# arnauqb/GradABM-JUNE

Hardware: AMD Instinct MI355X
Metric: simulation steps/sec (higher is better)
Workload: dtype f32

## Files before the change

gradabm-june_amd/csrc/gj_tiled.h:

```cpp
#pragma once
#include <hip/hip_runtime.h>
#include <stdint.h>

#include <type_traits>

#include "../../include/gradjune_hip.h"
#include "gj_device.h"

namespace gj {

constexpr int kTileThreads = 1024;
constexpr int kTileWaves = kTileThreads / kWave;
constexpr int kMaxSliceAgents = 19840;
constexpr int kUnroll = 8;
#ifndef GJ_UNROLL_NARROW
#define GJ_UNROLL_NARROW 16
#endif
constexpr int kUnrollNarrow = GJ_UNROLL_NARROW;
#ifndef GJ_VENUE_UNROLL
#define GJ_VENUE_UNROLL 2
#endif
constexpr int kVenueUnroll = GJ_VENUE_UNROLL;
#ifndef GJ_VENUE_UNROLL_C
#define GJ_VENUE_UNROLL_C GJ_VENUE_UNROLL
#endif
constexpr int kVenueUnrollC = GJ_VENUE_UNROLL_C;
#ifndef GJ_CUM_BATCH
#define GJ_CUM_BATCH 8
#endif
constexpr int kCumBatch = GJ_CUM_BATCH;

typedef unsigned long long fx_t;
template <int BITS>
__device__ __forceinline__ constexpr float fx_max() { return (float)(1ull << (50 - BITS)); }
template <int BITS>
__device__ __forceinline__ fx_t to_fx(float x) {
  constexpr double scale = (double)(1ull << BITS);
  constexpr double magic = 6755399441055744.0;
  const double d = __builtin_fma((double)x, scale, magic);
  return (fx_t)(__double_as_longlong(d) - 0x4338000000000000LL);
}
template <int BITS>
__device__ __forceinline__ float from_fx(fx_t v) {
  return (float)((double)(long long)v * (1.0 / (double)(1ull << BITS)));
}
constexpr float kSaturated = 1.0e30f;
__device__ __forceinline__ void fx_flag(uint32_t* flags, int words, int i, float x) {
  const uint32_t bit = 1u << (i & 31);
  if (!(x < 0.0f)) atomicOr(&flags[i >> 5], bit);
  if (!(x > 0.0f)) atomicOr(&flags[words + (i >> 5)], bit);
}
__device__ __forceinline__ float fx_special(uint32_t pos, uint32_t neg, float v) {
  return (pos & neg) ? __builtin_nanf("") : (pos ? kSaturated : (neg ? -kSaturated : v));
}
template <int BITS>
__device__ __forceinline__ float fx_read(const fx_t* sums, const uint32_t* flags, int words, int i) {
  const uint32_t pos = (flags[i >> 5] >> (i & 31)) & 1u, neg = (flags[words + (i >> 5)] >> (i & 31)) & 1u;
  return fx_special(pos, neg, from_fx<BITS>(sums[i]));
}
constexpr int kFxVenue = 36, kFxAgent = 32;
__device__ __forceinline__ uint32_t abs_bits(float x) { return __float_as_uint(x) & 0x7FFFFFFFu; }
template <int N>
__device__ __forceinline__ uint32_t max_abs_bits(const float (&x)[N]) {
  uint32_t m = 0u;
#pragma unroll
  for (int q = 0; q < N; ++q) m = max(m, abs_bits(x[q]));
  return m;
}
template <int BITS>
constexpr uint32_t fx_limit_bits() { return (uint32_t)(127 + 50 - BITS) << 23; }
constexpr uint32_t kAgentLimitBits = fx_limit_bits<kFxAgent>();
static_assert(kAgentLimitBits == 0x48800000u, "the pattern of fx_max<kFxAgent>() = 262144.0f");

template <typename T>
__device__ __forceinline__ T* elem32(T* base, int idx) {
  using Byte = typename std::conditional<std::is_const<T>::value, const char, char>::type;
  return reinterpret_cast<T*>(reinterpret_cast<Byte*>(base) + (uint64_t)((uint32_t)idx * (uint32_t)sizeof(T)));
}
template <typename T>
__device__ __forceinline__ T at32(const T* base, int idx) { return *elem32(base, idx); }
template <typename T>
__device__ __forceinline__ void put32(T* base, int idx, T v) { *elem32(base, idx) = v; }

typedef float gj_v4f __attribute__((ext_vector_type(4)));
typedef unsigned int gj_v4u __attribute__((ext_vector_type(4)));
typedef unsigned int gj_v2u __attribute__((ext_vector_type(2)));
template <typename T>
__device__ __forceinline__ T at32nt(const T* base, int idx) { return __builtin_nontemporal_load(elem32(base, idx)); }
template <typename T>
__device__ __forceinline__ void put32nt(T* base, int idx, T v) { __builtin_nontemporal_store(v, elem32(base, idx)); }
__device__ __forceinline__ uint4 load_nt(const uint4* p) {
  const gj_v4u v = __builtin_nontemporal_load(reinterpret_cast<const gj_v4u*>(p));
  return make_uint4(v.x, v.y, v.z, v.w);
}
__device__ __forceinline__ float4 load_nt(const float4* p) {
  const gj_v4f v = __builtin_nontemporal_load(reinterpret_cast<const gj_v4f*>(p));
  return make_float4(v.x, v.y, v.z, v.w);
}
__device__ __forceinline__ void store_nt(float4* p, float4 x) {
  gj_v4f v = {x.x, x.y, x.z, x.w};
  __builtin_nontemporal_store(v, reinterpret_cast<gj_v4f*>(p));
}
struct TSetA {
  const uint16_t* a_la;
  const int32_t* tile_sptr;
  const int32_t* tile_jpos;
  const int32_t* chunk_ptr;
  const int4* chunk_desc;
  float* val;
  int32_t J;
  int32_t active;
  int32_t raw;
  int32_t wide;
  int32_t direct;
  int32_t presum;
  const int32_t* multi_slots;
};

struct TileAArgs {
  TSetA sets[GJ_MAX_SETS];
  int32_t n_sets;
  int32_t slice_agents;
  int64_t n_agents;
  const float* trans;
  const float* qtrans;
};

__device__ __forceinline__ void load_slice(float* lds, const float* __restrict__ src, int64_t base, int n_local,
                                           int tid) {
  const int n4 = n_local >> 2;
  const float4* s4 = reinterpret_cast<const float4*>(src + base);
  float4* d4 = reinterpret_cast<float4*>(lds);
  constexpr int kQ = (kMaxSliceAgents + 4 * kTileThreads - 1) / (4 * kTileThreads);
  if (n4 > 0) {
    float4 v[kQ];
#pragma unroll
    for (int u = 0; u < kQ; ++u) v[u] = s4[min(tid + u * kTileThreads, n4 - 1)];
#pragma unroll
    for (int u = 0; u < kQ; ++u)
      if (tid + u * kTileThreads < n4) d4[tid + u * kTileThreads] = v[u];
  }
  for (int i = (n4 << 2) + tid; i < n_local; i += kTileThreads) lds[i] = src[base + i];
}

__device__ __forceinline__ int chunk_slot_fast(const int4 d, int lane) {
  const int split = d.z & 0xFFFF;
  return (lane < split) ? d.x + lane : d.y + (lane - split);
}
__device__ __noinline__ int chunk_slot_slow(const TSetA& T, const int4 d, int row, int i, int lane) {
  const int split = d.z & 0xFFFF;
  if (lane < split) return d.x + lane;
  int j = d.w;
  while (i >= T.tile_sptr[row + j + 1]) ++j;
  return T.tile_jpos[row + j] + (i - T.tile_sptr[row + j]);
}

__device__ __forceinline__ int chunk_slot_wide(const int4 d0, const int4 d1, int lane) {
  int b = d0.x;
  b = (lane >= (d1.z & 0xFF)) ? d0.y : b;
  b = (lane >= ((d1.z >> 8) & 0xFF)) ? d0.z : b;
  b = (lane >= ((d1.z >> 16) & 0xFF)) ? d0.w : b;
  b = (lane >= ((d1.z >> 24) & 0xFF)) ? d1.x : b;
  b = (lane >= (d1.w & 0xFF)) ? d1.y : b;
  return b + lane;
}
__device__ __noinline__ int chunk_slot_walk(const TSetA& T, int row, int i, int j) {
  while (i >= T.tile_sptr[row + j + 1]) ++j;
  return T.tile_jpos[row + j] + (i - T.tile_sptr[row + j]);
}

struct Segment {
  int row, seg0, seg1, c_base, n_chunks;
  __device__ __forceinline__ Segment(const TSetA& T, int s)
      : row(s * T.J), seg0(T.tile_sptr[row]), seg1(T.tile_sptr[row + T.J]), c_base(T.chunk_ptr[s]),
        n_chunks(T.chunk_ptr[s + 1] - c_base) {}
  __device__ __forceinline__ int edge(int c, int u, int lane) const { return seg0 + (c + u) * kWave + lane; }
  __device__ __forceinline__ bool has(int c, int u, int lane) const { return (c + u < n_chunks) && (edge(c, u, lane) < seg1); }
  __device__ __forceinline__ int edge_clamped(int c, int u, int lane) const { return min(edge(c, u, lane), seg1 - 1); }
};
// ... 120 lines not shown
    scatter_batches<WIDE, kUnroll>(T, lds_x, s, wave, lane);
  }
}

template <int kU>
__device__ __forceinline__ void agent_add_batch(fx_t* lds_acc, uint32_t* lds_flags, int flag_words, const int (&la)[kU],
                                                const float (&x)[kU]) {
  if (__builtin_expect(max_abs_bits(x) <= kAgentLimitBits, 1)) {
#pragma unroll
    for (int u = 0; u < kU; ++u) atomicAdd(&lds_acc[la[u]], to_fx<kFxAgent>(x[u]));
  } else {
#pragma unroll
    for (int u = 0; u < kU; ++u) {
      if (abs_bits(x[u]) <= kAgentLimitBits) {
        atomicAdd(&lds_acc[la[u]], to_fx<kFxAgent>(x[u]));
      } else {
        fx_flag(lds_flags, flag_words, la[u], x[u]);
      }
    }
  }
}

#ifndef GJ_UNROLL_D_NARROW
#define GJ_UNROLL_D_NARROW 8
#endif
template <bool WIDE>
__device__ __forceinline__ void gather_set(const TSetA& T, fx_t* lds_acc, uint32_t* lds_flags, int flag_words, int s,
                                           int wave, int lane) {
  const Segment G(T, s);
  constexpr int kU = WIDE ? kUnroll : GJ_UNROLL_D_NARROW;
  constexpr int kStride = kTileWaves * kU;
  auto stage1 = [&](int c, int& word, int (&la)[kU]) { batch_stage1<WIDE, kU>(T, G, c, lane, word, la); };
  auto values = [&](int c, int word, float (&v)[kU]) {
    int slot[kU];
    batch_slots<WIDE, kU>(T, G, word, c, lane, slot);
#pragma unroll
    for (int u = 0; u < kU; ++u) v[u] = at32nt(T.val, G.has(c, u, lane) ? slot[u] : 0);
  };
  auto add = [&](int c, const int (&la)[kU], const float (&v)[kU]) {
    float x[kU];
#pragma unroll
    for (int u = 0; u < kU; ++u) x[u] = G.has(c, u, lane) ? v[u] : 0.0f;
    agent_add_batch<kU>(lds_acc, lds_flags, flag_words, la, x);
  };
  int c0 = wave * kU;
  if (c0 >= G.n_chunks) return;
  int laA[kU], wordA;
  float v[kU];
  int laB[kU], wordB;
  stage1(c0, wordA, laA);
  while (true) {
    const int c1 = c0 + kStride;
    values(c0, wordA, v);
    stage1(c1, wordB, laB);
    add(c0, laA, v);
    if (c1 >= G.n_chunks) break;
    const int c2 = c1 + kStride;
    values(c1, wordB, v);
    stage1(c2, wordA, laA);
    add(c1, laB, v);
    if (c2 >= G.n_chunks) break;
    c0 = c2;
  }
}

template <int kU>
__device__ __forceinline__ void explicit_stage1(const TSetA& T, const Segment G, int c0, int lane, int (&la)[kU], int (&sl)[kU]) {
  const int32_t* slots = reinterpret_cast<const int32_t*>(T.chunk_desc);
#pragma unroll
  for (int u = 0; u < kU; ++u) {
    const int i = G.edge_clamped(c0, u, lane);
    la[u] = at32(T.a_la, i);
    sl[u] = at32(slots, i);
  }
}
template <int kU>
__device__ __forceinline__ void scatter_explicit(const TSetA& T, const float* lds_x, int s, int wave, int lane) {
  const Segment G(T, s);
  for (int c0 = wave * kU; c0 < G.n_chunks; c0 += kTileWaves * kU) {
    int la[kU], sl[kU];
    explicit_stage1<kU>(T, G, c0, lane, la, sl);
#pragma unroll
    for (int u = 0; u < kU; ++u)
      if (G.has(c0, u, lane)) put32(T.val, sl[u], lds_x[la[u]]);
  }
}

template <int kU>
__device__ __forceinline__ void gather_explicit(const TSetA& T, fx_t* lds_acc, uint32_t* lds_flags, int flag_words, int s,
                                                int wave, int lane) {
  const Segment G(T, s);
  for (int c0 = wave * kU; c0 < G.n_chunks; c0 += kTileWaves * kU) {
    int la[kU], sl[kU];
    explicit_stage1<kU>(T, G, c0, lane, la, sl);
    float x[kU];
#pragma unroll
    for (int u = 0; u < kU; ++u) x[u] = at32(T.val, sl[u]);
#pragma unroll
    for (int u = 0; u < kU; ++u) x[u] = G.has(c0, u, lane) ? x[u] : 0.0f;
    agent_add_batch<kU>(lds_acc, lds_flags, flag_words, la, x);
  }
}

#ifndef GJ_SCATTER_WAVES_PER_SIMD
#define GJ_SCATTER_WAVES_PER_SIMD 4
#endif
__global__ __launch_bounds__(kTileThreads, GJ_SCATTER_WAVES_PER_SIMD) void k_tile_scatter(const TileAArgs A) {
  extern __shared__ __align__(16) float lds_x[];
  const int tid = threadIdx.x;
  const int wave = __builtin_amdgcn_readfirstlane(tid / kWave), lane = tid % kWave;
  const int s = blockIdx.x;
  const int64_t base = (int64_t)s * A.slice_agents;
  const int n_local = (int)min((int64_t)A.slice_agents, A.n_agents - base);
  const bool two_sources = A.qtrans != A.trans;
  for (int pass = 0; pass < 2; ++pass) {
    if (pass == 1 && !two_sources) break;
    bool any = false;
    for (int t = 0; t < A.n_sets; ++t)
      if (A.sets[t].active && !A.sets[t].presum && (!two_sources || A.sets[t].raw == pass)) any = true;
    if (!any) continue;
    if (pass == 1) __syncthreads();
    load_slice(lds_x, pass == 0 ? A.qtrans : A.trans, base, n_local, tid);
    __syncthreads();
    for (int t = 0; t < A.n_sets; ++t) {
      const TSetA& T = A.sets[t];
      if (!T.active || T.presum || (two_sources && T.raw != pass)) continue;
      if (T.wide == 2) {
        scatter_explicit<kUnroll>(T, lds_x, s, wave, lane);
      } else if (T.wide) {
        scatter_set<true>(T, lds_x, s, wave, lane);
      } else {
        scatter_set<false>(T, lds_x, s, wave, lane);
      }
    }
  }
}

struct TSetB {
  const int32_t* blk_v0;
  const int32_t* blk_e0;
  const uint16_t* e_lv;
  const uint8_t* e_cls;
  float* val;
  const float* v_pc;
  float* cum;
  int32_t stride;
  int32_t nk;
  float beta[GJ_MAX_NETS_PER_SET];
  int32_t table[GJ_MAX_NETS_PER_SET];
  int32_t age75[GJ_MAX_NETS_PER_SET];
  int32_t leisure;
  int32_t direct;
  uint32_t term_limit;
  int32_t _pad_b;
  const uint16_t* pv_blk;
  const int32_t* blk_r0;
  const float* x;
  int64_t n_x;
};

struct TileBArgs {
  TSetB sets[GJ_MAX_SETS];
  const int32_t* work;
  const float* tables;
  int32_t day_type;
  int32_t mode;
  int32_t transpose;
  int32_t _pad;
};

struct ClassWeights {
  float l, lw;
};
__device__ __forceinline__ ClassWeights class_weights(const float* tables, int table, int age75, int day_type, int c) {
  const float l = tables[(int64_t)table * GJ_TABLE_SIZE + day_type * 200 + c];
  return {l, age75 ? l * (((c % 100) > 75) ? 1.0f : 0.0f) : l};
}
template <bool TRANSMITTING, bool RECEIVING, typename TSet>
__device__ __forceinline__ void fill_class_weights(float* transmitting, float* receiving, const TSet& T, const float* tables,
                                                   int day_type, int transpose, int tid) {
  for (int i = tid; i < T.nk * 200; i += kTileThreads) {
    const int k = i / 200, c = i % 200;
    const ClassWeights w = class_weights(tables, T.table[k], T.age75[k], day_type, c);
    if (TRANSMITTING) transmitting[i] = transpose ? w.lw : w.l;
    if (RECEIVING) receiving[i] = transpose ? w.l : w.lw;
  }
}

__device__ __noinline__ void venue_group_slow(fx_t* sums, uint32_t* vflags, int words, uint32_t limit, int base_k, int l0,
                                              int l1, int l2, int l3, int l4, int l5, int l6, int l7, float x0, float x1,
                                              float x2, float x3, float x4, float x5, float x6, float x7) {
  const int lv[8] = {l0, l1, l2, l3, l4, l5, l6, l7};
  const float x[8] = {x0, x1, x2, x3, x4, x5, x6, x7};
#pragma unroll
  for (int q = 0; q < 8; ++q) {
    if (lv[q] == 0xFFFF) continue;
    if (abs_bits(x[q]) <= limit) {
      atomicAdd(&sums[base_k + lv[q]], to_fx<kFxVenue>(x[q]));
    } else {
      fx_flag(vflags, words, base_k + lv[q], x[q]);
    }
  }
}

__device__ __forceinline__ int class_byte(uint32_t four, int j) { return (four >> (8 * j)) & 0xFF; }

struct Group8 {
  uint32_t w[4], c[2];
  float v[8];
  __device__ __forceinline__ Group8(uint4 raw, uint2 craw, float4 xa = make_float4(0.0f, 0.0f, 0.0f, 0.0f),
                                    float4 xb = make_float4(0.0f, 0.0f, 0.0f, 0.0f))
      : w{raw.x, raw.y, raw.z, raw.w}, c{craw.x, craw.y}, v{xa.x, xa.y, xa.z, xa.w, xb.x, xb.y, xb.z, xb.w} {}
  __device__ __forceinline__ int lv(int q) const { return (w[q >> 1] >> ((q & 1) * 16)) & 0xFFFF; }
  __device__ __forceinline__ float x(int q) const { return v[q]; }
  __device__ __forceinline__ int cls(int q) const { return class_byte(c[q >> 2], q & 3); }
  __device__ __forceinline__ void drop(int q) { w[q >> 1] |= 0xFFFFu << ((q & 1) * 16); }
  __device__ __forceinline__ bool one_venue() const {
    return (w[0] == w[1]) && (w[1] == w[2]) && (w[2] == w[3]) && ((w[0] >> 16) == (w[0] & 0xFFFFu)) && (lv(0) != 0xFFFF);
  }
  __device__ __forceinline__ Group8 weighted(const float* tk) const {
    Group8 g = *this;
#pragma unroll
    for (int q = 0; q < 8; ++q) g.v[q] = tk[cls(q)] * v[q];
    return g;
  }
};

#ifdef GJ_DIAG_STAMPS
constexpr int kDiagVenueSlots = 8192;
__device__ unsigned long long gj_diag_venue[3 * kDiagVenueSlots];
struct VenueStamp {
  unsigned long long t0;
  __device__ VenueStamp() : t0(__builtin_amdgcn_s_memrealtime()) {}
  __device__ ~VenueStamp() {
    if (threadIdx.x == 0 && blockIdx.x < kDiagVenueSlots) {
      gj_diag_venue[3 * blockIdx.x] = t0;
      gj_diag_venue[3 * blockIdx.x + 1] = __builtin_amdgcn_s_memrealtime();
      gj_diag_venue[3 * blockIdx.x + 2] = __builtin_amdgcn_s_getreg((31 << 11) | 20) & 0xF;
    }
  }
};
#else
struct VenueStamp {};
#endif

struct VenueItem {
  const TSetB& T;
  int tid, nk;
  int v0, nv;
  int g0, g1;
  fx_t* sums;
  float* cumf;
  float* tabs;
  uint32_t* vflags;
  int vwords;
  int dummy;
  __device__ __forceinline__ VenueItem(const TSetB& T_, int j, float* lds, int tid_)
      : T(T_), tid(tid_), nk(T_.nk), v0(T_.blk_v0[j]), nv(T_.blk_v0[j + 1] - v0), g0(T_.blk_e0[j] >> 3),
        g1(T_.blk_e0[j + 1] >> 3), sums(reinterpret_cast<fx_t*>(lds)), cumf(lds), tabs(lds + 2 * ((size_t)nk * nv + 64)),
        vflags(reinterpret_cast<uint32_t*>(tabs + (T_.leisure ? 2 * nk * 200 : 0))), vwords((nk * nv + 64 + 31) / 32),
        dummy(nk * nv + (tid_ & 63)) {}
  __device__ __forceinline__ const uint4* lv8() const { return reinterpret_cast<const uint4*>(T.e_lv); }
  __device__ __forceinline__ const uint2* cls8() const { return reinterpret_cast<const uint2*>(T.e_cls); }
  __device__ __forceinline__ float4* val4() const { return reinterpret_cast<float4*>(T.val); }
};

__device__ __forceinline__ void run_sums(const VenueItem& W, const Group8& G, int base_k, fx_t* sums, uint32_t* vflags) {
  const uint32_t kLimit = W.T.term_limit;
  static_assert(kFxVenue == 36, "term_limit is derived from 2^(50 - kFxVenue) (fill_set_b)");
  if (__builtin_expect(max_abs_bits(G.v) > kLimit, 0)) {
    venue_group_slow(sums, vflags, W.vwords, kLimit, base_k, G.lv(0), G.lv(1), G.lv(2), G.lv(3), G.lv(4), G.lv(5),
                     G.lv(6), G.lv(7), G.x(0), G.x(1), G.x(2), G.x(3), G.x(4), G.x(5), G.x(6), G.x(7));
    return;
  }
  fx_t s8 = 0;
#pragma unroll
  for (int q = 0; q < 8; ++q) {
    const fx_t f = to_fx<kFxVenue>(G.x(q));
    const bool first = (q == 0) || (G.lv(q) != G.lv(q - (q > 0)));
    s8 = first ? f : s8 + f;
    const bool last = (q == 7) || (G.lv(q + (q < 7)) != G.lv(q));
    const bool take = last && G.lv(q) != 0xFFFF;
    atomicAdd(&sums[take ? base_k + G.lv(q) : W.dummy], s8);
  }
}
__device__ __forceinline__ bool one_venue_sum(const VenueItem& W, const Group8& G, int target, fx_t* sums) {
  if (__builtin_amdgcn_ballot_w64(max_abs_bits(G.v) > W.T.term_limit) != 0ull) return false;
  fx_t s = 0;
#pragma unroll
  for (int q = 0; q < 8; ++q) s += to_fx<kFxVenue>(G.x(q));
  s = wave_sum<fx_t>(s);
  if ((W.tid & (kWave - 1)) == 0) atomicAdd(&sums[target], s);
  return true;
}

__device__ __forceinline__ void venue_zero(const VenueItem& W, fx_t* sums, uint32_t* vflags) {
  for (int i = W.tid; i < W.nk * W.nv + 64; i += kTileThreads) sums[i] = 0;
  for (int i = W.tid; i < 2 * W.vwords; i += kTileThreads) vflags[i] = 0u;
}

__device__ __forceinline__ void venue_sums_tiled(const VenueItem& W, const float* weights, fx_t* sums, uint32_t* vflags) {
  const TSetB& T = W.T;
  auto add_group = [&](const Group8& G) {
    const bool mine = G.one_venue() && (G.lv(0) == __builtin_amdgcn_readfirstlane(G.lv(0)));
    const bool one_venue = __builtin_amdgcn_ballot_w64(mine) == ~0ull;
    if (!T.leisure) {
      if (!(one_venue && one_venue_sum(W, G, G.lv(0), sums))) run_sums(W, G, 0, sums, vflags);
    } else {
      for (int k = 0; k < W.nk; ++k) {
        const Group8 Gk = G.weighted(weights + k * 200);
        if (!(one_venue && one_venue_sum(W, Gk, k * W.nv + G.lv(0), sums))) run_sums(W, Gk, k * W.nv, sums, vflags);
      }
    }
  };
  for (int g = W.g0 + W.tid; g < W.g1; g += kVenueUnroll * kTileThreads) {
    uint4 raw[kVenueUnroll];
    float4 xa[kVenueUnroll], xb[kVenueUnroll];
    uint2 craw[kVenueUnroll];
#pragma unroll
    for (int u = 0; u < kVenueUnroll; ++u) {
      const int gu = min(g + u * kTileThreads, W.g1 - 1);
      raw[u] = W.lv8()[gu];
      xa[u] = load_nt(W.val4() + 2 * gu);
      xb[u] = load_nt(W.val4() + 2 * gu + 1);
      craw[u] = T.leisure ? W.cls8()[gu] : make_uint2(0u, 0u);
    }
#pragma unroll
    for (int u = 0; u < kVenueUnroll; ++u)
      if (g + u * kTileThreads < W.g1) add_group(Group8(raw[u], craw[u], xa[u], xb[u]));
  }
}

__device__ __forceinline__ void venue_sums_runs(const VenueItem& W, int j, fx_t* sums, uint32_t* vflags) {
  const TSetB& T = W.T;
  const int r0 = T.blk_r0[j], r1 = T.blk_r0[j + 1];
  const uint4* pv8 = reinterpret_cast<const uint4*>(T.pv_blk);
  const float4* x4 = reinterpret_cast<const float4*>(T.x);
  const int ga = r0 >> 3, gb = (r1 + 7) >> 3;
  const int g_in = (int)(T.n_x >> 3);
  for (int g = ga + W.tid; g < gb; g += kVenueUnroll * kTileThreads) {
    uint4 raw[kVenueUnroll];
    float4 xa[kVenueUnroll], xb[kVenueUnroll];
#pragma unroll
    for (int u = 0; u < kVenueUnroll; ++u) {
      const int gu = min(g + u * kTileThreads, gb - 1);
      raw[u] = pv8[gu];
      if (gu < g_in) {
        xa[u] = x4[2 * gu];
        xb[u] = x4[2 * gu + 1];
      } else {
        float t[8];
#pragma unroll
        for (int q = 0; q < 8; ++q) t[q] = ((int64_t)gu * 8 + q < T.n_x) ? T.x[(int64_t)gu * 8 + q] : 0.0f;
        xa[u] = make_float4(t[0], t[1], t[2], t[3]);
        xb[u] = make_float4(t[4], t[5], t[6], t[7]);
      }
    }
#pragma unroll
    for (int u = 0; u < kVenueUnroll; ++u) {
      const int gu = g + u * kTileThreads;
      if (gu >= gb) continue;
      Group8 G(raw[u], make_uint2(0u, 0u), xa[u], xb[u]);
#pragma unroll
      for (int q = 0; q < 8; ++q) {
        const int a = gu * 8 + q;
        if (!(a >= r0 && a < r1)) G.drop(q);
      }
      run_sums(W, G, 0, sums, vflags);
    }
  }
}

__device__ __forceinline__ void venue_cum_write(const VenueItem& W, const fx_t* sums, const uint32_t* vflags, float* cumf) {
  const TSetB& T = W.T;
  for (int l0 = W.tid; l0 < W.nv; l0 += kCumBatch * kTileThreads) {
    float pc[kCumBatch];
#pragma unroll
    for (int u = 0; u < kCumBatch; ++u) pc[u] = T.v_pc[W.v0 + min(l0 + u * kTileThreads, W.nv - 1)];
    for (int k = 0; k < W.nk; ++k) {
      const float beta = T.beta[k];
#pragma unroll
      for (int u = 0; u < kCumBatch; ++u) {
        const int lv = l0 + u * kTileThreads;
        if (lv < W.nv) {
          const float c = (beta * pc[u]) * fx_read<kFxVenue>(sums, vflags, W.vwords, k * W.nv + lv);
          T.cum[(int64_t)(W.v0 + lv) * T.stride + k] = c;
          cumf[2 * (k * W.nv + lv)] = c;
        }
      }
    }
  }
}
__device__ __forceinline__ void venue_cum_read(const VenueItem& W, float* cumf) {
  const TSetB& T = W.T;
  for (int k = 0; k < W.nk; ++k) {
    for (int l0 = W.tid; l0 < W.nv; l0 += kCumBatch * kTileThreads) {
      float c[kCumBatch];
#pragma unroll
      for (int u = 0; u < kCumBatch; ++u)
        c[u] = T.cum[(int64_t)(W.v0 + min(l0 + u * kTileThreads, W.nv - 1)) * T.stride + k];
#pragma unroll
      for (int u = 0; u < kCumBatch; ++u) {
        const int lv = l0 + u * kTileThreads;
        if (lv < W.nv) cumf[2 * (k * W.nv + lv)] = c[u];
      }
    }
  }
}

__device__ __forceinline__ void venue_gather(const VenueItem& W, const float* weights, const float* cumf) {
  const TSetB& T = W.T;
  const int nk = W.nk, nv = W.nv;
  for (int g = W.g0 + W.tid; g < W.g1; g += kVenueUnrollC * kTileThreads) {
    uint4 raw[kVenueUnrollC];
    uint2 craw[kVenueUnrollC];
#pragma unroll
    for (int u = 0; u < kVenueUnrollC; ++u) {
      const int gu = min(g + u * kTileThreads, W.g1 - 1);
      raw[u] = W.lv8()[gu];
      craw[u] = T.leisure ? W.cls8()[gu] : make_uint2(0u, 0u);
    }
#pragma unroll
    for (int u = 0; u < kVenueUnrollC; ++u) {
      const int gu = g + u * kTileThreads;
      if (gu >= W.g1) continue;
      const Group8 G(raw[u], craw[u]);
      float r[8];
      if (!T.leisure) {
#pragma unroll
        for (int q = 0; q < 8; ++q) {
          const int lv = G.lv(q);
          const float c = cumf[2 * (lv != 0xFFFF ? lv : 0)];
          r[q] = (lv != 0xFFFF) ? c : 0.0f;
        }
      } else {
#pragma unroll
        for (int q = 0; q < 8; ++q) {
          const int lv = G.lv(q);
          const int c = G.cls(q);
          const int li = lv != 0xFFFF ? lv : 0;
          float a = 0.0f;
          for (int k = 0; k < nk; ++k) a += weights[k * 200 + c] * cumf[2 * (k * nv + li)];
          r[q] = (lv != 0xFFFF) ? a : 0.0f;
        }
      }
      store_nt(W.val4() + 2 * gu, make_float4(r[0], r[1], r[2], r[3]));
      store_nt(W.val4() + 2 * gu + 1, make_float4(r[4], r[5], r[6], r[7]));
    }
  }
}

#ifndef GJ_VENUE_WAVES_PER_SIMD
#define GJ_VENUE_WAVES_PER_SIMD 4
#endif
__global__ __launch_bounds__(kTileThreads, GJ_VENUE_WAVES_PER_SIMD) void k_tile_venues(const TileBArgs B) {
  extern __shared__ __align__(16) float lds_s[];
  [[maybe_unused]] const VenueStamp gj_stamp;
  const int set = B.work[2 * blockIdx.x], j = B.work[2 * blockIdx.x + 1];
  const TSetB& T = B.sets[set];
  if (T.nk == 0) return;
  const VenueItem W(T, j, lds_s, threadIdx.x);
  if (T.leisure) fill_class_weights<true, true>(W.tabs, W.tabs + W.nk * 200, T, B.tables, B.day_type, B.transpose, W.tid);
  if (B.mode != 2) {
    venue_zero(W, W.sums, W.vflags);
    __syncthreads();
    venue_sums_tiled(W, W.tabs, W.sums, W.vflags);
    if (T.pv_blk) venue_sums_runs(W, j, W.sums, W.vflags);
    __syncthreads();
    venue_cum_write(W, W.sums, W.vflags, W.cumf);
    if (B.mode == 1 || T.direct) return;
  } else {
    if (T.direct) return;
    venue_cum_read(W, W.cumf);
  }
  __syncthreads();
  venue_gather(W, W.tabs + W.nk * 200, W.cumf);
}

constexpr int GJ_MAX_PRESUM = 6;
constexpr int64_t kPresumBad = (int64_t)0x8000000000000000ll;
struct TPSet {
  const uint16_t* ell;
  int64_t plane_stride;
  fx_t* partial;
  int32_t planes, V, stride, nk;
  int32_t group_venues;
  int32_t raw, leisure, _pad;
  int32_t table[GJ_MAX_NETS_PER_SET];
  int32_t age75[GJ_MAX_NETS_PER_SET];
};
struct TilePArgs {
  TPSet sets[GJ_MAX_PRESUM];
  int32_t n_sets;
  int32_t agents_per_wg;
  int64_t n_agents;
  const float* trans;
  const float* qtrans;
  const uint8_t* cls;
  const float* tables;
  int32_t day_type, transpose;
};

constexpr int kPresumQuads = 3;
__device__ __forceinline__ void fx_add_or_poison(fx_t* sums, uint32_t* flags, int i, float x) {
  const bool ok = fabsf(x) <= fx_max<kFxVenue>();
  atomicAdd(&sums[i], to_fx<kFxVenue>(ok ? x : 0.0f));
  if (__builtin_expect(!ok, 0)) atomicOr(&flags[i >> 5], 1u << (i & 31));
}

__global__ __launch_bounds__(kTileThreads) void k_tile_presum(const TilePArgs P) {
  extern __shared__ __align__(16) fx_t lds_p[];
  const int tid = threadIdx.x;
  const int64_t a_begin = (int64_t)blockIdx.x * P.agents_per_wg;
  const int64_t a_end = min(P.n_agents, a_begin + P.agents_per_wg);
  const int n_quads = (int)((max(a_end - a_begin, (int64_t)0) + 3) >> 2);
  for (int t = 0; t < P.n_sets; ++t) {
    const TPSet& T = P.sets[t];
    const int nk = T.nk;
    const float* x = T.raw ? P.trans : P.qtrans;
    for (int v0 = 0; v0 < T.V; v0 += T.group_venues) {
      const int nv = min(T.group_venues, T.V - v0);
      const int n_sums = nv * nk;
      const int dummy = n_sums + (tid & 63);
      float* wtab = reinterpret_cast<float*>(lds_p + n_sums + 64);
      uint32_t* flags = reinterpret_cast<uint32_t*>(wtab + (T.leisure ? nk * 200 : 0));
      __syncthreads();
      for (int i = tid; i < n_sums + 64; i += kTileThreads) lds_p[i] = 0;
      for (int i = tid; i < (n_sums + 64 + 31) / 32; i += kTileThreads) flags[i] = 0u;
      if (T.leisure) fill_class_weights<true, false>(wtab, nullptr, T, P.tables, P.day_type, P.transpose, tid);
      __syncthreads();
      for (int plane = 0; plane < T.planes; ++plane) {
        const uint16_t* ell = T.ell + plane * T.plane_stride + a_begin * 2;
        struct Batch {
          uint4 rows[kPresumQuads];
          float4 xs[kPresumQuads];
          uint32_t cl[kPresumQuads];
        };
        auto load = [&](int b0, Batch& B) {
#pragma unroll
          for (int u = 0; u < kPresumQuads; ++u) {
            const int q = min(b0 + tid + u * kTileThreads, n_quads - 1);
            const int64_t a0 = a_begin + 4 * (int64_t)q;
            B.rows[u] = *reinterpret_cast<const uint4*>(ell + 8 * (int64_t)q);
            if (a0 + 4 <= P.n_agents) {
              B.xs[u] = *reinterpret_cast<const float4*>(x + a0);
            } else {
              B.xs[u] = make_float4(a0 < P.n_agents ? x[a0] : 0.0f, a0 + 1 < P.n_agents ? x[a0 + 1] : 0.0f,
                                    a0 + 2 < P.n_agents ? x[a0 + 2] : 0.0f, 0.0f);
            }
            B.cl[u] = T.leisure ? *reinterpret_cast<const uint32_t*>(P.cls + a0) : 0u;
          }
        };
        auto add = [&](int b0, const Batch& B) {
#pragma unroll
          for (int u = 0; u < kPresumQuads; ++u) {
            const int q = b0 + tid + u * kTileThreads;
            if (q >= n_quads) continue;
            const uint32_t w[4] = {B.rows[u].x, B.rows[u].y, B.rows[u].z, B.rows[u].w};
            const float xv[4] = {B.xs[u].x, B.xs[u].y, B.xs[u].z, B.xs[u].w};
            const int n_ok = (int)min((int64_t)4, a_end - (a_begin + 4 * (int64_t)q));
#pragma unroll
            for (int j = 0; j < 4; ++j) {
#pragma unroll
              for (int c = 0; c < 2; ++c) {
                const int lv = (int)((w[j] >> (16 * c)) & 0xFFFF) - v0;
                const bool in = ((unsigned)lv < (unsigned)nv) && (j < n_ok);
                if (!T.leisure) {
                  fx_add_or_poison(lds_p, flags, in ? lv : dummy, in ? xv[j] : 0.0f);
                } else {
                  const int cj = class_byte(B.cl[u], j);
                  for (int k = 0; k < nk; ++k)
                    fx_add_or_poison(lds_p, flags, in ? lv * nk + k : dummy, in ? wtab[k * 200 + cj] * xv[j] : 0.0f);
                }
              }
            }
          }
        };
        constexpr int kStep = kPresumQuads * kTileThreads;
        if (n_quads > 0) {
          Batch ba, bb;
          int b0 = 0;
          load(b0, ba);
          while (true) {
            const bool more1 = b0 + kStep < n_quads;
            if (more1) load(b0 + kStep, bb);
            add(b0, ba);
            if (!more1) break;
            b0 += kStep;
            const bool more2 = b0 + kStep < n_quads;
            if (more2) load(b0 + kStep, ba);
            add(b0, bb);
            if (!more2) break;
            b0 += kStep;
          }
        }
      }
      __syncthreads();
      fx_t* out = T.partial + (int64_t)blockIdx.x * T.V * T.stride;
      for (int i = tid; i < n_sums; i += kTileThreads) {
        const int lv = i / nk, k = i % nk;
        const bool bad = (flags[i >> 5] >> (i & 31)) & 1u;
        out[(int64_t)(v0 + lv) * T.stride + k] = bad ? (fx_t)kPresumBad : lds_p[i];
      }
    }
  }
}

struct PReduceSet {
  const fx_t* partial;
  const float* v_pc;
  float* cum;
  int32_t V, stride, nk, first;
  float beta[GJ_MAX_NETS_PER_SET];
};
struct PReduceArgs {
  PReduceSet sets[GJ_MAX_PRESUM];
  int32_t n_sets, n_wgs;
  int32_t total;
// ... 574 lines not shown
```

gradabm-june_amd/csrc/gradjune_hip.hip:

```cpp
#include <hip/hip_runtime.h>
#include <math.h>
#include <stdint.h>
#include <string.h>

#include "../../include/gradjune_hip.h"
#include "gj_device.h"
#include "gj_tiled.h"
#include "gj_agent.h"
#include "gj_location.h"

namespace gj {

struct SetP1 {
  const int32_t* v_rowptr;
  const int32_t* v_agent;
  const float* v_pc;
  float* cum;
  int32_t stride;
  int32_t nk;
  float beta[GJ_MAX_NETS_PER_SET];
  int32_t table[GJ_MAX_NETS_PER_SET];
  int32_t raw;
  int32_t leisure;
};
// ... 753 lines not shown
  if (C.leisure && !classes_by_dword(plan)) return GJ_E_PLAN;
  return check_group(C);
}

static int tiled_presum(const gj_plan* plan, const gj_agent_state* st, const gj_step_params* p, const Groups& G,
                        hipStream_t stream) {
  const gj_tiled* T = plan->tiled;
  TilePArgs P;
  P.n_sets = 0;
  for (int g = 0; g < G.n; ++g) {
    if (!uses_presum(plan, G.set[g])) continue;
    if (P.n_sets == GJ_MAX_PRESUM) return GJ_E_PLAN;
    const int rc = presum_fill(plan, p, G, g, &P.sets[P.n_sets++]);
    if (rc) return rc;
  }
  if (P.n_sets == 0 || plan->n_agents == 0) return GJ_OK;
  const int64_t budget = 160 * 1024;
  size_t lds = 0;
  for (int t = 0; t < P.n_sets; ++t) {
    TPSet& X = P.sets[t];
    const int64_t fixed = 64 * 8 + (X.leisure ? (int64_t)X.nk * 200 * 4 : 0) + 64;
    int64_t per_venue = (int64_t)X.nk * 8;
    int64_t gv = (budget - fixed) * 8 / (per_venue * 8 + X.nk);
    if (T->direct_table_floats > 0 && gv > T->direct_table_floats / X.nk) gv = T->direct_table_floats / X.nk;
    if (gv > X.V) gv = X.V;
    if (gv < 1) gv = 1;
    X.group_venues = (int32_t)gv;
    const size_t need = (size_t)(gv * X.nk + 64) * 8 + (X.leisure ? (size_t)X.nk * 200 * 4 : 0) + ((size_t)(gv * X.nk + 64 + 31) / 32) * 4;
    if (need > lds) lds = need;
  }
  int64_t apw = (plan->n_agents + T->presum_wgs - 1) / T->presum_wgs;
  apw = (apw + 63) / 64 * 64;
  P.agents_per_wg = (int32_t)apw;
  P.n_agents = plan->n_agents;
  P.trans = st->transmission;
  P.qtrans = p->has_quarantine ? st->q_transmission : st->transmission;
  if (!aligned16(P.trans, P.qtrans)) return GJ_E_PLAN;
  P.cls = plan->agent_class;
  P.tables = plan->tables;
  P.day_type = p->day_type;
  P.transpose = p->transpose;
  int rc = allow_lds(k_tile_presum, lds);
  if (rc) return rc;
  return launch(k_tile_presum, T->presum_wgs, kTileThreads, lds, stream, P);
}

static int tiled_presum_reduce(const gj_plan* plan, const gj_step_params* p, const Groups& G, hipStream_t stream) {
  const gj_tiled* T = plan->tiled;
  PReduceArgs R;
  R.n_sets = 0;
  R.n_wgs = T->presum_wgs;
  R._pad = 0;
  int64_t total = 0;
  for (int g = 0; g < G.n; ++g) {
    const int s = G.set[g];
    if (!uses_presum(plan, s)) continue;
    if (R.n_sets == GJ_MAX_PRESUM) return GJ_E_PLAN;
    PReduceSet& X = R.sets[R.n_sets++];
    const gj_edge_set& E = plan->sets[s];
    X.partial = reinterpret_cast<const fx_t*>(T->sets[s].presum);
    X.v_pc = E.v_pcontact;
    X.cum = E.cum;
    X.V = (int32_t)E.n_venues;
    X.stride = E.cum_stride;
    X.nk = G.nk[g];
    X.first = (int32_t)total;
    const NetGroup C = classify_group(p, G, g);
    memcpy(X.beta, C.beta, sizeof(X.beta));
    total += (int64_t)X.V * X.nk;
  }
  if (R.n_sets == 0 || total == 0) return GJ_OK;
  if (total > INT32_MAX) return GJ_E_RANGE;
  R.total = (int32_t)total;
  return launch(k_presum_reduce, grid_for(total, 0, kWave), kThreads, 0, stream, R);
}

static int tiled_scatter(const gj_plan* plan, const gj_agent_state* st, const gj_step_params* p, const Groups& G,
                         hipStream_t stream) {
  const gj_tiled* T = plan->tiled;
  if (plan->n_ext_agents == 0 || G.n == 0) return GJ_OK;
  TileAArgs A;
  fill_set_a(plan, p, G, A.sets);
  A.n_sets = plan->n_sets;
  A.slice_agents = T->slice_agents;
  A.n_agents = plan->n_ext_agents;
  A.trans = st->transmission;
  A.qtrans = p->has_quarantine ? st->q_transmission : st->transmission;
  const size_t lds = slice_lds(T, sizeof(float));
  int rc = allow_lds(k_tile_scatter, lds);
  if (rc) return rc;
  rc = launch(k_tile_scatter, T->n_slices, kTileThreads, lds, stream, A);
  if (rc) return rc;
  return tiled_presum(plan, st, p, G, stream);
}

static uint32_t venue_term_limit(int32_t max_venue_edges) {
  int e = 14;
  int64_t p2 = 4096;
  while (p2 < (int64_t)max_venue_edges && e > -20) {
    p2 <<= 1;
    --e;
  }
  const float lim = ldexpf(1.0f, e);
  uint32_t bits;
  memcpy(&bits, &lim, sizeof(bits));
  return bits;
}

static int tiled_venues(const gj_plan* plan, const gj_agent_state* st, const gj_step_params* p, const Groups& G, int mode,
                        hipStream_t stream) {
  const gj_tiled* T = plan->tiled;
  if (G.n == 0) return GJ_OK;
  if (T->n_work == 0) return mode == 2 ? GJ_OK : tiled_presum_reduce(plan, p, G, stream);
  TileBArgs B;
  for (int s = 0; s < GJ_MAX_SETS; ++s) B.sets[s] = TSetB{};
  size_t lds = 16;
  for (int g = 0; g < G.n; ++g) {
    const int s = G.set[g];
    const gj_tiled_set& S = T->sets[s];
    const gj_edge_set& E = plan->sets[s];
    TSetB& X = B.sets[s];
    X.blk_v0 = S.blk_v0;
    X.blk_e0 = S.blk_e0;
    X.e_lv = S.e_lv;
    X.e_cls = S.e_cls;
    X.val = S.val;
    X.v_pc = E.v_pcontact;
    X.cum = E.cum;
    X.stride = E.cum_stride;
    X.nk = S.n_blocks > 0 ? G.nk[g] : 0;
    if (uses_presum(plan, s)) X.nk = 0;
    X.direct = S.ell_k != 0;
    const NetGroup C = classify_group(p, G, g);
    X.leisure = C.leisure;
    memcpy(X.beta, C.beta, sizeof(X.beta));
    memcpy(X.table, C.table, sizeof(X.table));
    memcpy(X.age75, C.age75, sizeof(X.age75));
    if (C.leisure && !S.e_cls && E.n_edges > 0) return GJ_E_PLAN;
    if (const int rc = check_group(C)) return rc;
    X.pv_blk = nullptr;
    X.blk_r0 = nullptr;
    X.x = nullptr;
    X.n_x = 0;
    if (S.run_pv_blk && mode != 2) {
      if (X.leisure) return GJ_E_PLAN;
      X.x = (p->has_quarantine && !C.raw) ? st->q_transmission : st->transmission;
      if (!X.x) return GJ_E_NULL;
      if (!aligned16(X.x, S.run_pv_blk)) return GJ_E_PLAN;
      X.pv_blk = S.run_pv_blk;
      X.blk_r0 = S.run_blk_r0;
      X.n_x = plan->n_ext_agents;
    }
    const size_t n_sums = (size_t)X.nk * S.max_block_venues + 64;
    const size_t need = n_sums * sizeof(fx_t) + (X.leisure ? 2 * 200 * (size_t)X.nk : 0) * sizeof(float) +
                        2 * ((n_sums + 31) / 32 * 4);
    X.term_limit = venue_term_limit(S.max_venue_edges);
    if (X.nk && need > lds) lds = need;
  }
  B.work = T->work;
  B.tables = plan->tables;
  B.day_type = p->day_type;
  B.mode = mode;
  B.transpose = p->transpose;
  int rc = allow_lds(k_tile_venues, lds);
  if (rc) return rc;
  rc = launch(k_tile_venues, T->n_work, kTileThreads, lds, stream, B);
  if (rc || mode == 2) return rc;
  return tiled_presum_reduce(plan, p, G, stream);
}

static int tiled_agents(const gj_plan* plan, const gj_agent_state* st, const gj_step_params* p, const Groups& G,
                        const gj_step_io* io, int sample, hipStream_t stream) {
  const gj_tiled* T = plan->tiled;
  if (plan->n_agents == 0) return GJ_OK;
  TileDArgs D;
  fill_set_a(plan, p, G, D.sets);
  D.n_sets = plan->n_sets;
  D.slice_agents = T->slice_agents;
  D.n_agents = plan->n_agents;
  D.stage = st->current_stage;
  D.susceptibility = st->susceptibility;
  D.is_infected = st->is_infected;
  D.infection_time = st->infection_time;
  D.not_infected_probs = io ? io->not_infected_probs : nullptr;
  D.new_infected = io ? io->new_infected : nullptr;
  D.trans_susc = io ? io->trans_susc : nullptr;
  D.agent_sums = io ? io->agent_sums : nullptr;
  D.exp_noise = io ? io->exp_noise : nullptr;
  D.now = p->now;
  D.dt = p->delta_time;
  D.q_thr = p->q_threshold;
  D.has_q = p->has_quarantine;
  D.sample = sample;
  D.seed = p->seed;
  D.step = p->step;
  D.agent_offset = p->agent_offset;
  D.clock = p->clock;
  D.acc_scratch = T->agent_scratch;
  size_t lds = agents_lds(T);
  D.n_direct = 0;
  D.day_type = p->day_type;
  D.transpose = p->transpose;
  D.cls = plan->agent_class;
  D.tables = plan->tables;
  const int64_t owned_slices = (plan->n_agents + T->slice_agents - 1) / T->slice_agents;
  for (int g = 0; g < G.n; ++g) {
    const int s = G.set[g];
    const gj_tiled_set& S = T->sets[s];
    const gj_edge_set& E = plan->sets[s];
    const bool run = S.run_pv_win != nullptr;
    if ((!S.ell_k && !run) || S.n_blocks == 0 || E.n_edges == 0) continue;
    if (D.n_direct == GJ_MAX_DIRECT) return GJ_E_PLAN;
    TDirect& X = D.direct[D.n_direct++];
    X.ell = run ? S.run_pv_win : S.ell;
    X.cum = E.cum;
    X.planes = run ? 1 : S.ell_k / 2;
    X.plane_stride = owned_slices * (int64_t)T->slice_agents * 2;
    X.V = run ? S.run_max_window : (int32_t)E.n_venues;
    X.win_lo = run ? S.run_win_lo : nullptr;
    X.win_n = run ? S.run_win_n : nullptr;
    if (run && (uintptr_t)S.run_pv_win % 8 != 0) return GJ_E_PLAN;
    X.stride = E.cum_stride;
    const NetGroup C = classify_group(p, G, g);
    X.nk = C.nk;
    X.raw = C.raw;
    X.leisure = C.leisure;
    memcpy(X.table, C.table, sizeof(X.table));
    memcpy(X.age75, C.age75, sizeof(X.age75));
    if (C.leisure && !classes_by_dword(plan)) return GJ_E_PLAN;
    if (const int rc = check_group(C)) return rc;
  }
  D.table_floats = D.table1_floats = 0;
  D._pad3 = 0;
  if (D.n_direct) {
    const int64_t budget = 160 * 1024 / 4 - 2 * kClassWeightFloats - 2 * kWave;
    int64_t largest = 0;
    for (int t = 0; t < D.n_direct; ++t) {
      const int64_t sz = (int64_t)D.direct[t].V * D.direct[t].stride;
      largest = largest > sz ? largest : sz;
    }
    int64_t cap0 = largest < budget ? largest : budget;
    if (T->direct_table_floats > 0 && T->direct_table_floats < cap0) cap0 = T->direct_table_floats;
    if (cap0 < GJ_MAX_NETS_PER_SET) cap0 = GJ_MAX_NETS_PER_SET;
    int64_t cap1 = budget - cap0;
    if (T->direct_table_floats > 0 && T->direct_table_floats < cap1) cap1 = T->direct_table_floats;
    int prev_region = -1;
    for (int t = 0; t < D.n_direct; ++t) {
      TDirect& X = D.direct[t];
      const int64_t sz = (int64_t)X.V * X.stride;
      X.region = (prev_region == 0 && sz <= cap1) ? 1 : 0;
      const int64_t cap = X.region ? cap1 : cap0;
      X.group_venues = sz <= cap ? X.V : (int32_t)(cap / X.stride);
      if (X.group_venues < 1 || (X.win_lo && sz > cap)) return GJ_E_PLAN;
      prev_region = X.region;
    }
    D.table_floats = (int32_t)cap0;
    D.table1_floats = (int32_t)cap1;
    const size_t direct_lds = 4 * ((size_t)2 * kClassWeightFloats + (size_t)cap0 + kWave + (size_t)cap1 + kWave);
    if (direct_lds > lds) lds = direct_lds;
  }
  D.io_vec4 = aligned16(D.susceptibility, D.not_infected_probs, D.new_infected, D.trans_susc, D.acc_scratch, D.agent_sums);
  int rc = allow_lds(k_tile_agents, lds);
  if (rc) return rc;
  rc = launch(k_tile_agents, owned_slices, kTileThreads, lds, stream, D);
  if (rc || !D.acc_scratch) return rc;
  return launch(k_tile_epilogue, grid_for(plan->n_agents), kThreads, 0, stream, D);
}

static int check_symptoms(const uint8_t* agent_class, const float* new_infected, const float* current_stage,
                          const float* next_stage, const float* time_to_next_stage, const gj_symptoms_params* params,
                          const float* progresses, const float* dwell) {
  if (!agent_class || !new_infected || !current_stage || !next_stage || !time_to_next_stage || !params)
    return GJ_E_NULL;
  if (params->n_stages < 3 || params->n_stages > GJ_MAX_STAGES) return GJ_E_RANGE;
  if ((progresses == nullptr) != (dwell == nullptr)) return GJ_E_NULL;
  if (!progresses && !params->progress) return GJ_E_NULL;
  return GJ_OK;
}

static StatsArgs stats_args(int64_t n, const uint8_t* agent_class, const float* is_infected, const float* current_stage,
                            int32_t n_bins, const int32_t* bin_edges, int32_t dead_stage, double* out, bool vec4) {
  StatsArgs S;
  S.n = n;
  S.cls = agent_class;
  S.inf = is_infected;
  S.stage = current_stage;
  S.n_bins = n_bins;
  for (int b = 0; b <= GJ_MAX_AGE_BINS; ++b) S.edges[b] = (b <= n_bins) ? bin_edges[b] : 0;
  S.dead = dead_stage;
  S.vec4 = (vec4 && (uintptr_t)agent_class % 4 == 0) ? 1 : 0;
  S.out = out;
  return S;
}
static inline int64_t vec4_lanes(int64_t n, int vec4) { return vec4 ? (n >> 2) + 3 : n; }

static int check_profile_adjoint(const gj_agent_state* st, const float* trans_bar, const float* grad_inf_out,
                                 const float* grad_time_inout) {
  if (!st || !trans_bar || !grad_inf_out || !grad_time_inout) return GJ_E_NULL;
  if (!st->max_infectiousness || !st->shape || !st->rate || !st->shift || !st->infection_time || !st->is_infected)
    return GJ_E_NULL;
  return GJ_OK;
}

}


extern "C" {

// ... 664 lines not shown
```

Measured before the change: 1949.

## Compact nonzero venue contributions per wave before multi-net atomic accumulation

Adds a compacted venue-sum path for sets with two or more networks. Each wave ballots the live, nonzero agent entries, stages them in LDS, and then runs the per-network weighted atomics only over those entries, so zero or empty slots no longer each trigger nk rounds of atomic work. Groups with too many live entries, and leisure sets whose class weights are non-finite, fall back to the old path. This costs extra LDS per block, which can lower occupancy, plus ballot and staging overhead.

```diff
diff --git a/gradabm-june_amd/csrc/gj_tiled.h b/gradabm-june_amd/csrc/gj_tiled.h
--- a/gradabm-june_amd/csrc/gj_tiled.h
+++ b/gradabm-june_amd/csrc/gj_tiled.h
@@ -25,6 +25,17 @@
 #define GJ_VENUE_UNROLL_C GJ_VENUE_UNROLL
 #endif
 constexpr int kVenueUnrollC = GJ_VENUE_UNROLL_C;
+#ifndef GJ_VENUE_COMPACT
+#define GJ_VENUE_COMPACT 1
+#endif
+#ifndef GJ_VENUE_COMPACT_MAX
+#define GJ_VENUE_COMPACT_MAX 64
+#endif
+#ifndef GJ_VENUE_COMPACT_PLAIN
+#define GJ_VENUE_COMPACT_PLAIN 0
+#endif
+constexpr int kVenueCompactMinNets = GJ_VENUE_COMPACT ? (GJ_VENUE_COMPACT_PLAIN ? 1 : 2) : 0;
+constexpr size_t kVenueCompactLds = 4 * (size_t)kTileWaves + 8 * (size_t)kTileWaves * 8 * 64;
 #ifndef GJ_CUM_BATCH
 #define GJ_CUM_BATCH 8
 #endif
@@ -451,7 +462,7 @@
   int32_t leisure;
   int32_t direct;
   uint32_t term_limit;
-  int32_t _pad_b;
+  int32_t compact;
   const uint16_t* pv_blk;
   const int32_t* blk_r0;
   const float* x;
@@ -477,13 +488,25 @@
 }
 template <bool TRANSMITTING, bool RECEIVING, typename TSet>
 __device__ __forceinline__ void fill_class_weights(float* transmitting, float* receiving, const TSet& T, const float* tables,
-                                                   int day_type, int transpose, int tid) {
+                                                   int day_type, int transpose, int tid, uint32_t* nonfinite = nullptr) {
+  bool bad = false;
   for (int i = tid; i < T.nk * 200; i += kTileThreads) {
     const int k = i / 200, c = i % 200;
     const ClassWeights w = class_weights(tables, T.table[k], T.age75[k], day_type, c);
-    if (TRANSMITTING) transmitting[i] = transpose ? w.lw : w.l;
+    if (TRANSMITTING) {
+      const float t = transpose ? w.lw : w.l;
+      transmitting[i] = t;
+      bad |= abs_bits(t) >= 0x7F800000u;
+    }
     if (RECEIVING) receiving[i] = transpose ? w.l : w.lw;
   }
+  if (nonfinite) {
+    const bool any = __builtin_amdgcn_ballot_w64(bad) != 0ull;
+    if ((tid & (kWave - 1)) == 0) nonfinite[tid / kWave] = any ? 1u : 0u;
+  }
+}
+__device__ __forceinline__ bool weights_nonfinite(const uint32_t* nonfinite, int tid) {
+  return __builtin_amdgcn_ballot_w64(nonfinite[tid & (kTileWaves - 1)] != 0u) != 0ull;
 }
 
 __device__ __noinline__ void venue_group_slow(fx_t* sums, uint32_t* vflags, int words, uint32_t limit, int base_k, int l0,
@@ -598,20 +621,23 @@
   for (int i = W.tid; i < 2 * W.vwords; i += kTileThreads) vflags[i] = 0u;
 }
 
+__device__ __forceinline__ void venue_add_group(const VenueItem& W, const float* weights, fx_t* sums, uint32_t* vflags,
+                                                const Group8& G) {
+  const TSetB& T = W.T;
+  const bool mine = G.one_venue() && (G.lv(0) == __builtin_amdgcn_readfirstlane(G.lv(0)));
+  const bool one_venue = __builtin_amdgcn_ballot_w64(mine) == ~0ull;
+  if (!T.leisure) {
+    if (!(one_venue && one_venue_sum(W, G, G.lv(0), sums))) run_sums(W, G, 0, sums, vflags);
+  } else {
+    for (int k = 0; k < W.nk; ++k) {
+      const Group8 Gk = G.weighted(weights + k * 200);
+      if (!(one_venue && one_venue_sum(W, Gk, k * W.nv + G.lv(0), sums))) run_sums(W, Gk, k * W.nv, sums, vflags);
+    }
+  }
+}
 __device__ __forceinline__ void venue_sums_tiled(const VenueItem& W, const float* weights, fx_t* sums, uint32_t* vflags) {
   const TSetB& T = W.T;
-  auto add_group = [&](const Group8& G) {
-    const bool mine = G.one_venue() && (G.lv(0) == __builtin_amdgcn_readfirstlane(G.lv(0)));
-    const bool one_venue = __builtin_amdgcn_ballot_w64(mine) == ~0ull;
-    if (!T.leisure) {
-      if (!(one_venue && one_venue_sum(W, G, G.lv(0), sums))) run_sums(W, G, 0, sums, vflags);
-    } else {
-      for (int k = 0; k < W.nk; ++k) {
-        const Group8 Gk = G.weighted(weights + k * 200);
-        if (!(one_venue && one_venue_sum(W, Gk, k * W.nv + G.lv(0), sums))) run_sums(W, Gk, k * W.nv, sums, vflags);
-      }
-    }
-  };
+  auto add_group = [&](const Group8& G) { venue_add_group(W, weights, sums, vflags, G); };
   for (int g = W.g0 + W.tid; g < W.g1; g += kVenueUnroll * kTileThreads) {
     uint4 raw[kVenueUnroll];
     float4 xa[kVenueUnroll], xb[kVenueUnroll];
@@ -629,6 +655,80 @@
       if (g + u * kTileThreads < W.g1) add_group(Group8(raw[u], craw[u], xa[u], xb[u]));
   }
 }
+
+#if GJ_VENUE_COMPACT
+constexpr int kStageRow = 8 * kWave;
+constexpr int kVenueCompactMax = GJ_VENUE_COMPACT_MAX;
+static_assert(kVenueCompactMax <= kStageRow, "a sparse row must fit the staging row");
+__device__ __forceinline__ void venue_sums_compact(const VenueItem& W, const float* weights, fx_t* sums, uint32_t* vflags,
+                                                   uint2* stage_all) {
+  const TSetB& T = W.T;
+  const uint32_t limit = T.term_limit;
+  const int lane = W.tid & (kWave - 1);
+  const int wave0 = __builtin_amdgcn_readfirstlane(W.tid - lane);
+  uint2* stage = stage_all + wave0 * 8;
+  for (int gw = W.g0 + wave0; gw < W.g1; gw += kVenueUnroll * kTileThreads) {
+    const int g = gw + lane;
+    uint4 raw[kVenueUnroll];
+    float4 xa[kVenueUnroll], xb[kVenueUnroll];
+    uint2 craw[kVenueUnroll];
+#pragma unroll
+    for (int u = 0; u < kVenueUnroll; ++u) {
+      const int gu = min(g + u * kTileThreads, W.g1 - 1);
+      raw[u] = W.lv8()[gu];
+      xa[u] = load_nt(W.val4() + 2 * gu);
+      xb[u] = load_nt(W.val4() + 2 * gu + 1);
+      craw[u] = T.leisure ? W.cls8()[gu] : make_uint2(0u, 0u);
+    }
+#pragma unroll
+    for (int u = 0; u < kVenueUnroll; ++u) {
+      const bool valid = g + u * kTileThreads < W.g1;
+      const Group8 G(raw[u], craw[u], xa[u], xb[u]);
+      bool live[8];
+      unsigned long long m[8];
+      int n = 0;
+#pragma unroll
+      for (int q = 0; q < 8; ++q) {
+        live[q] = valid && G.lv(q) != 0xFFFF && abs_bits(G.x(q)) != 0u;
+        m[q] = __builtin_amdgcn_ballot_w64(live[q]);
+        n += __builtin_popcountll(m[q]);
+      }
+      if (n == 0) continue;
+      if (n > kVenueCompactMax) {
+        if (valid) venue_add_group(W, weights, sums, vflags, G);
+        continue;
+      }
+      int base = 0;
+#pragma unroll
+      for (int q = 0; q < 8; ++q) {
+        if (m[q] == 0ull) continue;
+        const int off = __builtin_amdgcn_mbcnt_hi((uint32_t)(m[q] >> 32), __builtin_amdgcn_mbcnt_lo((uint32_t)m[q], base));
+        if (live[q]) stage[off] = make_uint2(__float_as_uint(G.x(q)), (uint32_t)G.lv(q) | ((uint32_t)G.cls(q) << 16));
+        base += __builtin_popcountll(m[q]);
+      }
+      __builtin_amdgcn_fence(__ATOMIC_RELEASE, "workgroup");
+      __builtin_amdgcn_wave_barrier();
+      __builtin_amdgcn_fence(__ATOMIC_ACQUIRE, "workgroup");
+      for (int e = lane; e < n; e += kWave) {
+        const uint2 ent = stage[e];
+        const float x = __uint_as_float(ent.x);
+        const int lv = ent.y & 0xFFFF, cls = ent.y >> 16;
+        for (int k = 0; k < W.nk; ++k) {
+          const float term = T.leisure ? weights[k * 200 + cls] * x : x;
+          const int i = k * W.nv + lv;
+          if (__builtin_expect(abs_bits(term) <= limit, 1)) {
+            atomicAdd(&sums[i], to_fx<kFxVenue>(term));
+          } else {
+            fx_flag(vflags, W.vwords, i, term);
+          }
+        }
+      }
+      __builtin_amdgcn_fence(__ATOMIC_RELEASE, "workgroup");
+      __builtin_amdgcn_wave_barrier();
+    }
+  }
+}
+#endif
 
 __device__ __forceinline__ void venue_sums_runs(const VenueItem& W, int j, fx_t* sums, uint32_t* vflags) {
   const TSetB& T = W.T;
@@ -759,10 +859,22 @@
   const TSetB& T = B.sets[set];
   if (T.nk == 0) return;
   const VenueItem W(T, j, lds_s, threadIdx.x);
+#if GJ_VENUE_COMPACT
+  uint32_t* const wflags = W.vflags + 2 * W.vwords;
+  if (T.leisure)
+    fill_class_weights<true, true>(W.tabs, W.tabs + W.nk * 200, T, B.tables, B.day_type, B.transpose, W.tid,
+                                   T.compact ? wflags : nullptr);
+#else
   if (T.leisure) fill_class_weights<true, true>(W.tabs, W.tabs + W.nk * 200, T, B.tables, B.day_type, B.transpose, W.tid);
+#endif
   if (B.mode != 2) {
     venue_zero(W, W.sums, W.vflags);
     __syncthreads();
+#if GJ_VENUE_COMPACT
+    if (T.compact && !(T.leisure && weights_nonfinite(wflags, W.tid)))
+      venue_sums_compact(W, W.tabs, W.sums, W.vflags, reinterpret_cast<uint2*>(wflags + kTileWaves));
+    else
+#endif
     venue_sums_tiled(W, W.tabs, W.sums, W.vflags);
     if (T.pv_blk) venue_sums_runs(W, j, W.sums, W.vflags);
     __syncthreads();
diff --git a/gradabm-june_amd/csrc/gradjune_hip.hip b/gradabm-june_amd/csrc/gradjune_hip.hip
--- a/gradabm-june_amd/csrc/gradjune_hip.hip
+++ b/gradabm-june_amd/csrc/gradjune_hip.hip
@@ -929,8 +929,12 @@
       X.n_x = plan->n_ext_agents;
     }
     const size_t n_sums = (size_t)X.nk * S.max_block_venues + 64;
-    const size_t need = n_sums * sizeof(fx_t) + (X.leisure ? 2 * 200 * (size_t)X.nk : 0) * sizeof(float) +
-                        2 * ((n_sums + 31) / 32 * 4);
+    size_t need = n_sums * sizeof(fx_t) + (X.leisure ? 2 * 200 * (size_t)X.nk : 0) * sizeof(float) +
+                  2 * ((n_sums + 31) / 32 * 4);
+    if (kVenueCompactMinNets && X.nk >= kVenueCompactMinNets && need + kVenueCompactLds <= 160 * 1024) {
+      X.compact = 1;
+      need += kVenueCompactLds;
+    }
     X.term_limit = venue_term_limit(S.max_venue_edges);
     if (X.nk && need > lds) lds = need;
   }
```

New measurement: 1947. Within noise of the previous version (-0.1%).
